# ouc-ocean-group/RRNet

Hardware: AMD Instinct MI355X
Metric: images/sec (train step) (higher is better)
Workload: dtype f32; 1 GPU; RRNet hourglass-104 (2 stacks) train step, 1024x1024 synthetic VisDrone frames, fp32; per_gpu_batch=8, global_batch=8, k=1500, parallelism=dp1

## Files before the change

include/rrnet_hip_wino.h:

```cpp
#ifndef RRNET_HIP_WINO_H
#define RRNET_HIP_WINO_H

#include <stddef.h>

#ifdef __cplusplus
extern "C" {
#endif

#ifndef __HIP_INCLUDE_HIP_HIP_RUNTIME_API_H__
#ifndef RRNET_HIP_H
typedef struct ihipStream_t *hipStream_t;
#endif
#endif

#define RR_WINO_PLAN_INTS 11
int rr_conv_wino_plan(int math, int n, int h, int wd, int c, int k, int r, int s, int stride, int pad_h, int pad_w, int out_h,
                      int out_w, int flags, int *plan);
size_t rr_conv_wino_ws_bytes(int n, int h, int wd, int c, int k);
int rr_wino_filter(const float *w, float *u, int k, int c, hipStream_t stream);
int rr_wino_filter_batch(const long long *table, int nfilters, hipStream_t stream);
int rr_conv_wino_fprop(const float *x, const float *u, const float *bias, float *y, double *stat_slab, float *ws, size_t ws_bytes,
                       int n, int h, int wd, int c, int k, int relu, int accumulate, hipStream_t stream);
int rr_conv_wino_dgrad_bnsum(const float *dy, const float *u, float *dx, float *ws, size_t ws_bytes, int n, int h, int wd, int c,
                             int k, int accumulate, const float *prod_y, const float *prod_z, const float *prod_mean,
                             const float *prod_invstd, const float *prod_mask_scale, const float *prod_mask_shift, double *slab,
                             double *sums, hipStream_t stream);
int rr_wino_input(const float *x, float *v, int n, int h, int wd, int c, hipStream_t stream);
int rr_wino_gemm(const float *v, const float *u, float *m, long tiles, int c, int k, hipStream_t stream);

#ifdef __cplusplus
}
#endif
#endif
```

rrnet_amd/csrc/conv.hip:

```cpp
#include "conv_launch.h"
#include <hip/amd_detail/amd_hip_unsafe_atomics.h>

namespace {

typedef float f32x4 __attribute__((ext_vector_type(4)));
typedef float f32x16 __attribute__((ext_vector_type(16)));

__device__ float rr_zero16[4] = {0.f, 0.f, 0.f, 0.f};

constexpr int BM = 128;
constexpr int BK = 32;

struct ConvArgs {
    const float *src;
    const float *w;
    float *dst;
    const float *bias;
    double *stat_slab;
    const float *bs_y, *bs_z, *bs_mean, *bs_invstd, *bs_msc, *bs_msh;
    int bs_relu_bias;
    int N;
    int SH, SW, SC;
    int DH, DW, DC;
    int R, S, stride, pad_h, pad_w;
// ... 673 lines not shown
#pragma unroll
            for (int w = 0; w < WM; ++w) {
                d1 += sred[(w * BN + t) * 2 + 0];
                d2 += sred[(w * BN + t) * 2 + 1];
            }
            double *slab = a.stat_slab + (long)m_tile * 2 * a.DC;
            slab[n0 + t] = d1;
            slab[a.DC + n0 + t] = d2;
        }
    }
}

struct WgradArgs {
    const float *x;
    const float *dy;
    float *dw;
    const float *zero;
    int N, H, W, C, K, R, S, P, Q, stride, pad_h, pad_w;
    int M;
    int chunks_per_split;
    int mt, nt;
    const int *gate;
    int gate_max;
};

template <int BMW, int BN, bool A_SCALAR, bool B_SCALAR, int PIPE>
__global__ __launch_bounds__(256, PIPE == 3 ? 3 : 1) void conv_wgrad_kernel(const WgradArgs a)
{
    static_assert(PIPE == 0 || PIPE == 1 || PIPE == 3, "conv_wgrad_kernel: PIPE 0, 1 or 3");
    if (a.gate != nullptr && *a.gate <= a.gate_max) return;
    constexpr int TILES = (BMW / 32) * (BN / 32);
    constexpr int KS = TILES == 1 ? 4 : 1;
    constexpr int WN = TILES == 16 ? 2 : (BN / 32 >= 4 ? 4 : 1);
    constexpr int WM = 4 / (WN * KS);
    constexpr int TM = BMW / (WM * 32);
    constexpr int TN = BN / (WN * 32);
    constexpr int A_ELEMS = BK * BMW, B_ELEMS = BK * BN;
    constexpr int TPR_A = BMW / 4, RPP_A = 256 / TPR_A, AJ = BMW / 32;
    constexpr int TPR_B = BN / 4, RPP_B = 256 / TPR_B, BJ = BN / 32;

    extern __shared__ __align__(16) float lds[];
    constexpr int NBUF = PIPE == 3 ? 1 : 2;
    float *As = lds, *Bs = lds + NBUF * A_ELEMS;

    const int t = threadIdx.x, lane = t & 63, wave = t >> 6;
    const int wk = KS > 1 ? wave : 0;
    const int wm = KS > 1 ? 0 : wave / WN, wn = KS > 1 ? 0 : wave % WN;
    const int RS = a.R * a.S;
    int logical = xcd_remap(blockIdx.x, gridDim.x);
    const int tap = logical % RS; logical /= RS;
    const int n_tile = logical % a.nt; logical /= a.nt;
    const int m_tile = logical % a.mt;
    const int split = logical / a.mt;
    const int r = tap / a.S, s = tap - r * a.S;
    const int ko0 = m_tile * BMW, c0 = n_tile * BN;
    const int total_chunks = (a.M + BK - 1) / BK;
    const int kc_begin = split * a.chunks_per_split;
    int kc_end = kc_begin + a.chunks_per_split;
    if (kc_end > total_chunks) kc_end = total_chunks;
    if (kc_begin >= kc_end) return;

    f32x4 ra[AJ], rb[BJ];
    const int a_row = t / TPR_A, a_col = (t % TPR_A) * 4;
    const int b_row = t / TPR_B, b_col = (t % TPR_B) * 4;

    int bn_[BJ], bp_[BJ], bq_[BJ];
#pragma unroll
    for (int j = 0; j < BJ; ++j) {
        const long m = (long)kc_begin * BK + b_row + RPP_B * j;
        const int pq = a.P * a.Q;
        bn_[j] = (int)(m / pq);
        const int rem = (int)(m - (long)bn_[j] * pq);
        bp_[j] = rem / a.Q;
        bq_[j] = rem - bp_[j] * a.Q;
    }
    const bool a_ko_ok = ko0 + a_col < a.K;
    const bool b_c_ok = c0 + b_col < a.C;
// ... 96 lines not shown
        for (int q = 0; q < 4; ++q) {
            const int kr = 2 * (4 * g + q) + lh;
#pragma unroll
            for (int i = 0; i < TM; ++i) fa[q][i] = A[kr * BMW + (wm * TM + i) * 32 + lr];
#pragma unroll
            for (int j = 0; j < TN; ++j) fb[q][j] = B[kr * BN + (wn * TN + j) * 32 + lr];
        }
    };
    auto sub = [&](const float (&fa)[4][TM], const float (&fb)[4][TN], int q) {
#pragma unroll
        for (int i = 0; i < TM; ++i)
#pragma unroll
            for (int j = 0; j < TN; ++j)
                acc[i][j] = __builtin_amdgcn_mfma_f32_32x32x2f32(fa[q][i], fb[q][j], acc[i][j], 0, 0, 0);
        __builtin_amdgcn_sched_barrier(0);
    };
    auto make_srd = [](const float *p, long bytes) {
        const unsigned long long u = reinterpret_cast<unsigned long long>(p);
        const unsigned lo = __builtin_amdgcn_readfirstlane((unsigned)u);
        const unsigned hi = __builtin_amdgcn_readfirstlane((unsigned)(u >> 32));
        void *q = reinterpret_cast<void *>(((unsigned long long)hi << 32) | lo);
        return __builtin_amdgcn_make_buffer_rsrc(q, 0, __builtin_amdgcn_readfirstlane((int)bytes), 0x00020000);
    };
    const __amdgpu_buffer_rsrc_t rs_dy = make_srd(a.dy, (long)a.M * a.K * 4);
    const long x_shift = ALIGNED ? (long)a.pad_w * a.C * 4 : 0;
    const __amdgpu_buffer_rsrc_t rs_x = make_srd(reinterpret_cast<const float *>(reinterpret_cast<const char *>(a.x) - x_shift),
                                                 (long)a.N * a.H * a.W * a.C * 4 + x_shift);
    constexpr unsigned OOB = 0xFFFFFFF0u;
    int a_off[AJ], a_m[AJ];
#pragma unroll
    for (int j = 0; j < AJ; ++j) {
        a_m[j] = a_row + RPP_A * j;
        a_off[j] = (a_m[j] * a.K + ko0 + a_col) * 4;
    }
    const int a_step = BK * a.K * 4;
    const int rr_off = r - a.pad_h, ss_off = s - a.pad_w;
    constexpr unsigned FAR = 0x80000000u;
    int s_n = 0, s_p = 0, s_q0 = 0;
    unsigned a_voff[AJ], b_voff[BJ];
    int b_iw0[BJ];
    if constexpr (ALIGNED) {
        const int m0 = kc_begin * BK, pq = a.P * a.Q;
        s_n = m0 / pq;
        const int rem = m0 - s_n * pq;
        s_p = rem / a.Q;
        s_q0 = rem - s_p * a.Q;
#pragma unroll
        for (int j = 0; j < AJ; ++j) a_voff[j] = a_ko_ok ? (unsigned)a_off[j] : FAR;
#pragma unroll
// ... 218 lines not shown
{
    const long M = (long)n * p * q;
    return (size_t)((M + BM - 1) / BM) * 2 * k * sizeof(double);
}

int rr_conv_wino_gemm(const float *v, const float *u, float *m, long tiles, int c, int k, hipStream_t stream, const char *name)
{
    RR_CHECK_ARG(tiles > 0 && c > 0 && k > 0 && c % 4 == 0 && k % 4 == 0 && tiles * c * 4 < (1l << 31) && tiles * k * 4 < (1l << 31)
                 && (long)k * c * 4 < (1l << 31), "%s: bad GEMM geometry", name);
    ConvArgs a{};
    a.src = v; a.w = u; a.dst = m; a.zero = zero_page();
    a.N = 1; a.SH = 1; a.SW = (int)tiles; a.SC = c;
    a.DH = 1; a.DW = (int)tiles; a.DC = k;
    a.R = 1; a.S = 1; a.stride = 1; a.ksplit = 1;
    a.M = (int)tiles; a.Kg = c; a.wK = k; a.wC = c; a.dst32 = 1;
    a.batch_src = tiles * c; a.batch_w = (long)k * c; a.batch_dst = tiles * k;
    const int bn = k > 64 ? 128 : 64;
    const dim3 grid(rr_cdiv(tiles, BM) * rr_cdiv(k, bn), 16, 1);
    if (bn == 128)
        return rr_launch(conv_igemm_kernel<128, 0, false, BK, 2, false, false, true>, grid, 256, igemm_lds(128, false, 1), stream, a, name);
    return rr_launch(conv_igemm_kernel<64, 0, false, BK, 2, false, false, true>, grid, 256, igemm_lds(64, false, 1), stream, a, name);
}

int rr_conv_colstats(const float *y, long M, int C, double *slab, hipStream_t stream, const char *name)
{
    const int lanes = 256 / (C / 4);
    int sblocks = rr_cdiv(M, (long)lanes * 8);
    if (sblocks > 256) sblocks = 256;
    hipLaunchKernelGGL(colstats_kernel, dim3(sblocks), dim3(256), 0, stream, y, M, C, slab);
    RR_CHECK_LAUNCH(name);
    return RR_OK;
}

static int fprop_impl(const char *name, const float *x, const float *w, const float *bias, float *y, double *stat_slab,
                      int n, int h, int wd, int c, int k, int r, int s, int stride, int pad_h,
                      int pad_w, int relu, int accumulate, hipStream_t stream, const BnSumArgs *bs = nullptr, const int *gate = nullptr,
                      int gate_max = 0)
{
    const rr_plan::FpropPlan pl = rr_plan::fprop_plan(rr_plan::MATH_F32, {n, h, wd, c, k, r, s, stride, pad_h, pad_w, 0, 0},
                                                      {bias != nullptr, relu != 0, stat_slab != nullptr, rr_conv_link(bs), accumulate != 0, false});
    RR_CHECK_ARG(pl.refuse == nullptr, "%s: %s", name, pl.refuse);
    RR_CHECK_ARG(gate == nullptr || (!pl.rows && !pl.pos_major && bs == nullptr && pl.after == rr_plan::AFTER_NONE && !pl.zero_slab),
                 "%s: this shape does not launch the plain forward kernel alone: no gate", name);
    if (pl.rows) return rr_conv1x1_rows(x, w, bias, y, pl.M, c, k, relu, stream);
    ConvArgs a{};
    a.gate = gate; a.gate_max = gate_max;
// ... 285 lines not shown
```

rrnet_amd/csrc/conv_launch.h:

```cpp
#pragma once
#include "common.h"
#include "conv_plan.h"
#include "rrnet_hip.h"
#include "rrnet_hip_rows.h"

struct BnSumArgs {
    const float *y, *z, *mean, *invstd, *msc, *msh;
    double *slab;
    double *sums;
    int relu_bias;
    bool bn_ok(int c) const { return y && mean && invstd && slab && sums && (!msc == !msh) && c % 4 == 0 && c <= 1024; }
    bool relu_bias_ok(int c, int k) const { return z && slab && sums && c % 4 == 0 && k % 4 == 0 && c <= 1024; }
    template <typename A> void into(A &a) const
    {
        a.stat_slab = slab; a.bs_y = y; a.bs_z = z; a.bs_mean = mean; a.bs_invstd = invstd; a.bs_msc = msc; a.bs_msh = msh; a.bs_relu_bias = relu_bias;
    }
};

template <typename K, typename A>
inline int rr_launch(K kern, dim3 grid, int threads, size_t lds, hipStream_t stream, const A &args, const char *name)
{
    if (lds > 48 * 1024)
        RR_CHECK_HIP(hipFuncSetAttribute(reinterpret_cast<const void *>(kern), hipFuncAttributeMaxDynamicSharedMemorySize, (int)lds), name);
    hipLaunchKernelGGL(kern, grid, dim3(threads), lds, stream, args);
    RR_CHECK_LAUNCH(name);
    return RR_OK;
}

inline int rr_refuse(const char *name, const rr_plan::Refusal &r)
{
    char why[256];
    snprintf(why, sizeof(why), r.why, r.a[0], r.a[1], r.a[2], r.a[3], r.a[4]);
    rr_set_error("%s: %s", name, why);
    return RR_ERR_ARG;
}

inline int rr_conv_link(const BnSumArgs *bs) { return bs == nullptr ? rr_plan::LINK_NONE : (bs->relu_bias ? rr_plan::LINK_RELU_BIAS : rr_plan::LINK_BN); }

int rr_conv_colstats(const float *y, long M, int C, double *slab, hipStream_t stream, const char *name);

int rr_conv_wino_gemm(const float *v, const float *u, float *m, long tiles, int c, int k, hipStream_t stream, const char *name);

int rr_gated_zero(float *p, size_t bytes, const int *count, int max_rows, int when_rows, hipStream_t stream, const char *name);

inline int rr_conv_before_launch(const rr_plan::FpropPlan &pl, int n, int k, float *y, double *stat_slab, hipStream_t stream, const char *name)
{
    RR_CHECK_HIP(rr_zero2(pl.zero_dst ? y : nullptr, pl.zero_dst ? sizeof(float) * (size_t)pl.M * k : 0, pl.zero_slab ? stat_slab : nullptr,
                          pl.zero_slab ? rr_conv_stat_slab_bytes(n, pl.dh, pl.dw, k) : 0, stream), name);
    return RR_OK;
}

inline int rr_conv_after_launch(const rr_plan::FpropPlan &pl, const BnSumArgs *bs, int k, const float *y, double *stat_slab, hipStream_t stream,
                                const char *name)
{
    switch (pl.after) {
    case rr_plan::AFTER_REDUCE_SLAB: return rr_bn_reduce_slab(bs->slab, rr_cdiv(pl.M, rr_plan::BM), k, bs->sums, stream);
    case rr_plan::AFTER_BWD_REDUCE: return rr_bn_bwd_reduce(y, bs->z, bs->y, bs->mean, bs->invstd, bs->msc, bs->msh, bs->sums, pl.M, k, 1, stream);
    case rr_plan::AFTER_COLSTATS: return rr_conv_colstats(y, pl.M, k, stat_slab, stream, name);
    default: return RR_OK;
    }
}

struct DgradS1Geom { int p, q, pad_h, pad_w; };
inline int rr_dgrad_s1_geom(const char *name, int h, int wd, int r, int s, int pad_h, int pad_w, bool producer_ok, DgradS1Geom *g)
// ... 56 lines not shown
```

rrnet_amd/csrc/conv_plan.h:

```cpp
#pragma once
#include <stdlib.h>

namespace rr_plan {

enum { MATH_F32 = 0, MATH_BF16 = 1, MATH_F16X3 = 2 };
enum { FAM_CONV16 = 3 };
enum { LINK_NONE = 0, LINK_BN = 1, LINK_RELU_BIAS = 2 };
enum { AFTER_NONE = 0, AFTER_REDUCE_SLAB = 1, AFTER_BWD_REDUCE = 2, AFTER_COLSTATS = 3 };

constexpr int BM = 128;
constexpr int BK = 32;

inline int cdiv(long a, long b) { return (int)((a + b - 1) / b); }

inline int mid_tiles() { return 48; }
inline int small_tiles() { return 16; }

inline int pick_ksplit(int blocks, int nk)
{
    static int enabled = -1;
    if (enabled < 0) {
        const char *e = getenv("RR_CONV_SPLITK");
        enabled = (e && atoi(e) == 0) ? 0 : 1;
    }
// ... 341 lines not shown
    RR_PLAN_REFUSE(math != MATH_F32, "fp32 arithmetic only");
    RR_PLAN_REFUSE(!(g.r == 3 && g.s == 3 && g.stride == 1 && g.pad_h == 1 && g.pad_w == 1), "3x3, stride 1, pad 1 only");
    RR_PLAN_REFUSE(g.out_h > 0 || g.out_w > 0, "no explicit output size");
    RR_PLAN_REFUSE(!(g.c % 4 == 0 && g.k % 4 == 0), "C and K must be multiples of 4");
    RR_PLAN_REFUSE(f.strided_dst, "no strided destination");
    RR_PLAN_REFUSE(f.link == LINK_RELU_BIAS, "the conv + bias + ReLU link is not built on this route");
    RR_PLAN_REFUSE(f.link == LINK_BN && (f.bias || f.relu || f.stats || g.k > 1024), "a BatchNorm link: plain data gradient, at most 1024 channels");
    const long M = (long)g.n * g.h * g.w;
    p.th = (g.h + 1) / 2; p.tw = (g.w + 1) / 2;
    p.tiles = (long)g.n * p.th * p.tw;
    RR_PLAN_REFUSE(!(M * g.c * 4 < G2 && M * g.k * 4 < G2 && 9l * g.c * g.k * 4 < G2 && p.tiles * g.c * 4 < G2 && p.tiles * g.k * 4 < G2),
                   "tensors must stay below 2 GiB");
    p.bn = g.k > 64 ? 128 : 64;
    p.gemm_blocks = cdiv(p.tiles, BM) * cdiv(g.k, p.bn);
    p.out_x = cdiv(M, BM);
    p.out_y = cdiv(g.k / 4, 64);
    p.tiles_per_wg = cdiv(p.tiles, p.out_x);
    p.ws_bytes = 16l * p.tiles * ((long)g.c + g.k) * 4;
    if (M < WINO_MIN_PIXELS) { p.refuse = "fewer output pixels than the route's floor"; p.floor_only = 1; }
#undef RR_PLAN_REFUSE
    return p;
}

}
```

rrnet_amd/csrc/conv_wino.hip:

```cpp
#include "conv_launch.h"
#include "rrnet_hip_wino.h"

namespace {

typedef float f32x4 __attribute__((ext_vector_type(4)));

__device__ __forceinline__ __amdgpu_buffer_rsrc_t wino_srd(const void *p, long bytes)
{
    const unsigned long long u = reinterpret_cast<unsigned long long>(p);
    const unsigned lo = __builtin_amdgcn_readfirstlane((unsigned)u);
    const unsigned hi = __builtin_amdgcn_readfirstlane((unsigned)(u >> 32));
    void *q = reinterpret_cast<void *>(((unsigned long long)hi << 32) | lo);
    return __builtin_amdgcn_make_buffer_rsrc(q, 0, __builtin_amdgcn_readfirstlane((int)bytes), 0x00020000);
}
constexpr unsigned OOB = 0xFFFFFFF0u;
__device__ __forceinline__ f32x4 wino_load(__amdgpu_buffer_rsrc_t rs, unsigned off)
{
    return __builtin_bit_cast(f32x4, __builtin_amdgcn_raw_buffer_load_b128(rs, off, 0, 0));
}

struct WinoFilterRow { const float *w; float *u; long K, C; };

__global__ __launch_bounds__(256) void wino_filter_kernel(const WinoFilterRow *table, const WinoFilterRow one)
{
// ... 46 lines not shown
#pragma unroll
            for (int j = 0; j < 4; ++j) {
                const int ih = h0 + i, iw = w0 + j;
                const bool in = (unsigned)ih < (unsigned)H && (unsigned)iw < (unsigned)W;
                const unsigned off = in ? (unsigned)((((n * H + ih) * W + iw) * C + c) * 4) : OOB;
                d[i][j] = wino_load(rs, off);
            }
        f32x4 m[4][4];
#pragma unroll
        for (int j = 0; j < 4; ++j) {
            m[0][j] = d[0][j] - d[2][j];
            m[1][j] = d[1][j] + d[2][j];
            m[2][j] = d[2][j] - d[1][j];
            m[3][j] = d[1][j] - d[3][j];
        }
        float *vp = v + t * C + c;
        const long bs = tiles * C;
#pragma unroll
        for (int a = 0; a < 4; ++a) {
            *reinterpret_cast<f32x4 *>(vp + (4 * a + 0) * bs) = m[a][0] - m[a][2];
            *reinterpret_cast<f32x4 *>(vp + (4 * a + 1) * bs) = m[a][1] + m[a][2];
            *reinterpret_cast<f32x4 *>(vp + (4 * a + 2) * bs) = m[a][2] - m[a][1];
            *reinterpret_cast<f32x4 *>(vp + (4 * a + 3) * bs) = m[a][1] - m[a][3];
        }
    }
}

struct WinoOutArgs {
    const float *m;
    float *y;
    const float *bias;
    double *slab;
    const float *bs_y, *bs_z, *bs_mean, *bs_invstd, *bs_msc, *bs_msh;
    int H, W, K, TH, TW;
    long tiles, y_bytes;
    int per_wg, relu, accumulate;
};

template <bool LINK>
__global__ __launch_bounds__(256) void wino_output_kernel(const WinoOutArgs a)
{
    __shared__ double sred[rr_plan::WINO_OUT_LANES][64][8];
    const int t = threadIdx.x, cl = t & 63, tl = t >> 6;
    const int c = (blockIdx.y * 64 + cl) * 4;
    const bool c_ok = c < a.K;
    const int cm = c_ok ? c : 0;
// ... 112 lines not shown
        for (int e = 0; e < 4; ++e) {
            double r1 = 0.0, r2 = 0.0;
#pragma unroll
            for (int l = 0; l < rr_plan::WINO_OUT_LANES; ++l) { r1 += sred[l][cl][e]; r2 += sred[l][cl][4 + e]; }
            row[c + e] = r1;
            row[a.K + c + e] = r2;
        }
    }
}

int grid_for(long threads)
{
    long blocks = (threads + 255) / 256;
    return (int)(blocks > 256 * 64 ? 256 * 64 : (blocks < 1 ? 1 : blocks));
}

int run_filter(const WinoFilterRow *table, const WinoFilterRow &one, int nfilters, int blocks_x, hipStream_t stream, const char *name)
{
    hipLaunchKernelGGL(wino_filter_kernel, dim3(blocks_x, nfilters), dim3(256), 0, stream, table, one);
    RR_CHECK_LAUNCH(name);
    return RR_OK;
}

int run_input(const float *x, float *v, int n, int h, int wd, int c, const rr_plan::WinoPlan &pl, hipStream_t stream, const char *name)
{
    hipLaunchKernelGGL(wino_input_kernel, dim3(grid_for(pl.tiles * (c / 4))), dim3(256), 0, stream, x, v, h, wd, c, pl.th, pl.tw, pl.tiles,
                       (long)n * h * wd * c * 4);
    RR_CHECK_LAUNCH(name);
    return RR_OK;
}

int checked_plan(const char *name, int n, int h, int wd, int c, int k, const rr_plan::ConvFlags &f, size_t ws_bytes, rr_plan::WinoPlan *pl)
{
    *pl = rr_plan::wino_plan(rr_plan::MATH_F32, {n, h, wd, c, k, 3, 3, 1, 1, 1, 0, 0}, f);
    RR_CHECK_ARG(pl->refuse == nullptr || pl->floor_only, "%s: %s", name, pl->refuse);
    RR_CHECK_ARG(ws_bytes >= (size_t)pl->ws_bytes, "%s: workspace of %ld bytes needed (rr_conv_wino_ws_bytes)", name, pl->ws_bytes);
    return RR_OK;
}

int run_route(const char *name, const float *x, const float *u, float *y, float *ws, int n, int h, int wd, int c, int k,
              const rr_plan::WinoPlan &pl, WinoOutArgs &o, bool link, hipStream_t stream)
{
    float *v = ws, *m = ws + 16 * pl.tiles * c;
    if (int rc = run_input(x, v, n, h, wd, c, pl, stream, name)) return rc;
    if (int rc = rr_conv_wino_gemm(v, u, m, pl.tiles, c, k, stream, name)) return rc;
    o.m = m; o.y = y; o.y_bytes = (long)n * h * wd * k * 4; o.H = h; o.W = wd; o.K = k; o.TH = pl.th; o.TW = pl.tw; o.tiles = pl.tiles; o.per_wg = pl.tiles_per_wg;
    if (link) hipLaunchKernelGGL(wino_output_kernel<true>, dim3(pl.out_x, pl.out_y), dim3(256), 0, stream, o);
    else hipLaunchKernelGGL(wino_output_kernel<false>, dim3(pl.out_x, pl.out_y), dim3(256), 0, stream, o);
    RR_CHECK_LAUNCH(name);
    return RR_OK;
}

}

extern "C" int rr_conv_wino_plan(int math, int n, int h, int wd, int c, int k, int r, int s, int stride, int pad_h, int pad_w, int out_h,
                                 int out_w, int flags, int *plan)
{
    RR_CHECK_ARG(plan != nullptr && ((flags >> 8) & 3) <= rr_plan::LINK_RELU_BIAS, "rr_conv_wino_plan: bad arguments");
    const rr_plan::WinoPlan pl = rr_plan::wino_plan(math, {n, h, wd, c, k, r, s, stride, pad_h, pad_w, out_h, out_w},
                                                    {(flags & 1) != 0, (flags & 2) != 0, (flags & 4) != 0, (flags >> 8) & 3, (flags & 8) != 0,
                                                     (flags & 16) != 0});
    const int out[RR_WINO_PLAN_INTS] = {pl.refuse == nullptr, pl.floor_only, (int)(pl.tiles & 0x7fffffff), (int)(pl.tiles >> 31), pl.bn, pl.gemm_blocks, pl.out_x,
                                        pl.out_y, pl.tiles_per_wg, (int)(pl.ws_bytes & 0x7fffffff), (int)(pl.ws_bytes >> 31)};
    for (int i = 0; i < RR_WINO_PLAN_INTS; ++i) plan[i] = out[i];
    return RR_OK;
}

// ... 2 lines not shown
    if (n <= 0 || h <= 0 || wd <= 0 || c <= 0 || k <= 0) return 0;
    return (size_t)16 * n * ((h + 1) / 2) * ((wd + 1) / 2) * ((size_t)c + k) * sizeof(float);
}

extern "C" int rr_wino_filter_batch(const long long *table, int nfilters, hipStream_t stream)
{
    static_assert(sizeof(WinoFilterRow) == 4 * sizeof(long long), "rr_wino_filter_batch: four 64-bit words per filter");
    RR_CHECK_ARG(table != nullptr && nfilters >= 0 && nfilters < 65536, "rr_wino_filter_batch: bad arguments");
    if (nfilters == 0) return RR_OK;
    return run_filter(reinterpret_cast<const WinoFilterRow *>(table), WinoFilterRow{}, nfilters, 64, stream, "rr_wino_filter_batch");
}

extern "C" int rr_wino_filter(const float *w, float *u, int k, int c, hipStream_t stream)
{
    RR_CHECK_ARG(w != nullptr && u != nullptr && k > 0 && c > 0, "rr_wino_filter: bad arguments");
    return run_filter(nullptr, WinoFilterRow{w, u, k, c}, 1, grid_for((long)k * c), stream, "rr_wino_filter");
}

extern "C" int rr_wino_input(const float *x, float *v, int n, int h, int wd, int c, hipStream_t stream)
{
    rr_plan::WinoPlan pl;
    if (int rc = checked_plan("rr_wino_input", n, h, wd, c, c, {}, (size_t)-1, &pl)) return rc;
    RR_CHECK_ARG(x != nullptr && v != nullptr, "rr_wino_input: null argument");
    return run_input(x, v, n, h, wd, c, pl, stream, "rr_wino_input");
}

extern "C" int rr_wino_gemm(const float *v, const float *u, float *m, long tiles, int c, int k, hipStream_t stream)
{
    RR_CHECK_ARG(v != nullptr && u != nullptr && m != nullptr, "rr_wino_gemm: null argument");
    return rr_conv_wino_gemm(v, u, m, tiles, c, k, stream, "rr_wino_gemm");
}

extern "C" int rr_conv_wino_fprop(const float *x, const float *u, const float *bias, float *y, double *stat_slab, float *ws, size_t ws_bytes,
                                  int n, int h, int wd, int c, int k, int relu, int accumulate, hipStream_t stream)
{
    rr_plan::WinoPlan pl;
    if (int rc = checked_plan("rr_conv_wino_fprop", n, h, wd, c, k,
                              {bias != nullptr, relu != 0, stat_slab != nullptr, rr_plan::LINK_NONE, accumulate != 0, false}, ws_bytes, &pl))
        return rc;
    RR_CHECK_ARG(x != nullptr && u != nullptr && y != nullptr && ws != nullptr, "rr_conv_wino_fprop: null argument");
    WinoOutArgs o{};
    o.bias = bias; o.slab = stat_slab; o.relu = relu != 0; o.accumulate = accumulate != 0;
    return run_route("rr_conv_wino_fprop", x, u, y, ws, n, h, wd, c, k, pl, o, false, stream);
}

extern "C" int rr_conv_wino_dgrad_bnsum(const float *dy, const float *u, float *dx, float *ws, size_t ws_bytes, int n, int h, int wd, int c,
                                        int k, int accumulate, const float *prod_y, const float *prod_z, const float *prod_mean,
                                        const float *prod_invstd, const float *prod_mask_scale, const float *prod_mask_shift, double *slab,
                                        double *sums, hipStream_t stream)
{
    const char *name = "rr_conv_wino_dgrad_bnsum";
    const BnSumArgs bs{prod_y, prod_z, prod_mean, prod_invstd, prod_mask_scale, prod_mask_shift, slab, sums, 0};
    RR_CHECK_ARG(bs.bn_ok(c) && dy != nullptr && u != nullptr && dx != nullptr && ws != nullptr,
                 "%s: bad arguments (every tensor, the producer's tensors and the two buffers; C %% 4 == 0, C <= 1024)", name);
    rr_plan::WinoPlan pl;
    if (int rc = checked_plan(name, n, h, wd, k, c, {false, false, false, rr_plan::LINK_BN, accumulate != 0, false}, ws_bytes, &pl)) return rc;
    WinoOutArgs o{};
    o.slab = slab; o.accumulate = accumulate != 0;
    o.bs_y = prod_y; o.bs_z = prod_z; o.bs_mean = prod_mean; o.bs_invstd = prod_invstd; o.bs_msc = prod_mask_scale; o.bs_msh = prod_mask_shift;
    if (int rc = run_route(name, dy, u, dx, ws, n, h, wd, k, c, pl, o, true, stream)) return rc;
    return rr_bn_reduce_slab(slab, pl.out_x, c, sums, stream);
}
```

rrnet_amd/ops.py:

```python
import os
import sys
import threading
import types
import weakref

import torch

from rrnet_amd import _C

CL = torch.channels_last


class KernelTimer:

    def __init__(self, only=None, every=1):
        self.records = []
        self.bytes = {}
        self.only = only
        self.every = max(int(every), 1)
        self.seen = {}

    def launch(self, name, flops, fn, detail=None, nbytes=0.0):
        if self.only is not None and name not in self.only:
            return fn()
# ... 628 lines not shown
        tail = (link.y, z if link.use_z else None, link.mean, link.invstd, link.msc, link.msh, slab, link.sums) + tail
    _launch(name, flops, "rr_conv_dgrad_s1" + sfx, (dy, wt, out) + geo + tail, geo[:7] + (1,),
            4.0 * (dy.numel() + out.numel() * ((2 if geo[9] else 1) + (link is not None)) + w.numel()))


def _dgrad_s2(dy, w, out, geo, flops, bf, conv16):
    src = bf16_of(dy) if conv16 else dy
    wsub = torch.empty(w.numel(), dtype=torch.bfloat16 if conv16 else torch.float32, device=dy.device)
    sfx, tag, tail = _math_call(bf, dy, w)
    _launch("conv16_dgrad_s2" if conv16 else "conv_dgrad_s2" + tag, flops, "rr_conv16_dgrad_s2" if conv16 else "rr_conv_dgrad_s2" + sfx,
            (src, w, out) + geo + (wsub,) + tail, geo[:7] + (2,))


def _dgrad_fp32(dy, w, out, geo, flops, stride):
    n, h, wd, c, k = geo[:5]
    _launch(_igemm_name("dgrad", c, (k % 4 != 0) or (c % 4 != 0), n * h * wd, stride), flops, "rr_conv_dgrad",
            (dy, w, out) + geo[:7] + (stride,) + geo[7:], geo[:7] + (stride,))


_WINO = _C.Family("rrnet_hip_wino.h")
_CONV_WINO = os.environ.get("RR_CONV_WINO", "1") != "0"
_WINO_BELOW_FLOOR = False
_WINO_TAKES = {}
_WINO_PLAN_FN = []
_WINO_WS = {}
FLAT_BUFFERS = weakref.WeakSet()


def wino_takes(n, h, wd, c, k, r, s, stride, pad, bias=False, relu=False, stats=False, accumulate=False, link=False):
    if not _CONV_WINO:
        return False
    key = (n, h, wd, c, k, r, s, stride, pad[0], pad[1], int(bias) | int(relu) << 1 | int(stats) << 2 | int(accumulate) << 3 | int(link) << 8)
    hit = _WINO_TAKES.get(key)
    if hit is None:
        if not _WINO_PLAN_FN:
            f, (sig, _) = getattr(_C.lib(), "rr_conv_wino_plan"), _C.declared("rr_conv_wino_plan")
            f.restype, f.argtypes = sig[0], sig[1]
            _WINO_PLAN_FN.append(f)
        plan = (_C.c_int * 11)()
        _C.check(_WINO_PLAN_FN[0](MATH_F32, *key[:10], 0, 0, key[10], plan), "rr_conv_wino_plan")
        hit = _WINO_TAKES[key] = (bool(plan[0]), bool(plan[1]))
    return hit[0] or (hit[1] and _WINO_BELOW_FLOOR)


def _wino_ws(device, n, h, wd, c, k):
    need = _WINO.call("rr_conv_wino_ws_bytes", n, h, wd, c, k) // 4
    key = (device, torch.cuda.current_stream(device).cuda_stream)
    ws = _WINO_WS.get(key)
    if ws is None or ws.numel() < need:
        _WINO_WS[key] = None
        ws = _WINO_WS[key] = torch.empty(need, dtype=torch.float32, device=device)
    return ws


def _wino_filter(w, flipped, wt=None):
    for flat in FLAT_BUFFERS:
        u = flat.wino_view(w, flipped)
        if u is not None:
            return u
    k, c = w.shape[0], w.shape[1]
    src = _flipped_filter(w, wt, None, False)[0] if flipped else w
    u = torch.empty(16 * k * c, dtype=torch.float32, device=w.device)
    _WINO.call("rr_wino_filter", src, u, *((c, k) if flipped else (k, c)))
    return u


def _dgrad_wino(dy, w, out, geo, flops, wt, link=None, z=None):
    n, h, wd, c, k = geo[:5]
    u, ws = _wino_filter(w, True, wt), _wino_ws(dy.device, n, h, wd, k, c)
    nbytes = 4.0 * (dy.numel() + out.numel() * ((2 if geo[9] else 1) + (link is not None)) + w.numel()) + 2.0 * ws.numel() * 4.0
    if link is None:
        _launch("conv_dgrad<wino>", flops * 16.0 / 36.0, "rr_conv_wino_fprop",
                (dy, u, None, out, None, ws, ws.numel() * 4, n, h, wd, k, c, 0, geo[9]), geo[:7] + (1,), nbytes, call=_WINO.call)
        return
    slab = torch.empty(_C.call("rr_conv_stat_slab_bytes", n, h, wd, c) // 8, dtype=torch.float64, device=dy.device)
    link.sums, link.dz = _ZEROS.take(2 * c, dy.device), out
    _launch("conv_dgrad<wino>+bnsum", flops * 16.0 / 36.0, "rr_conv_wino_dgrad_bnsum",
            (dy, u, out, ws, ws.numel() * 4, n, h, wd, c, k, geo[9], link.y, z if link.use_z else None, link.mean, link.invstd, link.msc,
             link.msh, slab, link.sums), geo[:7] + (1,), nbytes, call=_WINO.call)


_ROWS = _C.Family("rrnet_hip_rows.h")
_CONV_ROWS = os.environ.get("RR_CONV_ROWS", "1") != "0"
_ROWS_MAX_SHARE = 8
_TARGETS_MAX_SHARE = 4


# ... 73 lines not shown

def conv_wgrad(x, dy, dw, stride=1, pad=(0, 0), explicit_out=False, algo_c=None):
    _C.require_cuda(x, dy, dw)
    assert (is_nhwc(x) or is_phantom(x)) and (is_nhwc(dy) or is_phantom(dy)) and is_nhwc(dw)
    n, c, h, wd = x.shape
    k, c2, r, s = dw.shape
    assert c == c2 and dy.shape[1] == k
    flops = 2.0 * dy.shape[0] * dy.shape[2] * dy.shape[3] * k * (c * r * s if algo_c is None else algo_c)
    if wgrad16_takes(x.shape, dy.shape, dw.shape, stride) and not explicit_out:
        x16, dy16 = bf16_of(x), bf16_of(dy)
        _launch("conv16_wgrad", flops, "rr_conv16_wgrad", (x16, dy16, dw, n, h, wd, c, k, r, s, stride, pad[0], pad[1]),
                (n, h, wd, c, k, r, s, stride))
        return dw
    listed = rows_side.now(dy) if not explicit_out and not is_phantom(x) and not is_phantom(dy) else None
    if listed is not None and _rows_shape_ok(dy, tuple(x.shape), tuple(dw.shape), stride):
        rows, count = listed[:2]
        args = (x, dy, dw, n, h, wd, c, k, r, s, pad[0], pad[1])
        max_rows = n * h * wd // _ROWS_MAX_SHARE
        _launch("conv_wgrad<rows>", 0.0, "rr_conv_wgrad_rows", args + (rows, count, max_rows), (n, h, wd, c, k, r, s, 1), call=_ROWS.call)
        _launch("conv_wgrad<dense>", 0.0, "rr_conv_wgrad_unless", args + (count, max_rows), (n, h, wd, c, k, r, s, 1), call=_ROWS.call)
        return dw
    x, dy = f32_of(x), f32_of(dy)
    bf = _bf16_ok(c, k, r, s, x, dy, pixels=dy.shape[0] * dy.shape[2] * dy.shape[3]) if wgrad_16bit_shape(c, k, r, s) else 0
    sfx, tag, wtail = _math_call(bf, x, dy)
    _launch("conv_wgrad<BN=%d>%s" % (128 if c > 32 else 32, tag), flops, "rr_conv_wgrad" + sfx,
            (x, dy, dw, n, h, wd, c, k, r, s, stride, pad[0], pad[1]) + ((dy.shape[2], dy.shape[3]) if explicit_out else (0, 0)) + wtail,
            (n, h, wd, c, k, r, s, stride))
    return dw


def _f32(n, device):
    return torch.empty(n, dtype=torch.float32, device=device)


class _ZeroPool:

    CHUNK = 128 * 1024

    def __init__(self):
        self.buf = {}

    def take(self, n, device):
        n8 = (n + 1) // 2 * 2
        key = (device.type, device.index, torch.cuda.current_stream(device).cuda_stream if device.type == "cuda" else 0)
        cur = self.buf.get(key)
        if cur is None or cur[1] + n8 > cur[0].numel():
# ... 1577 lines not shown
```

Measured before the change: 21.48 images/sec.

## Add Winograd F(2x2,3x3) weight-gradient path for fp32 3x3 stride-1 convolutions

Adds a Winograd weight-gradient route for 3x3, stride-1, pad-1 fp32 convolutions. It transforms input tiles and output-gradient tiles into 16 transformed slices, runs a batched 16-slice GEMM through a BATCH variant of the existing wgrad kernel, then folds the 4x4 results back into 3x3 filter gradients with accumulation. The aim is to cut the multiply count of the dominant wgrad GEMMs, paid for with extra transform passes, a large workspace, a zero-fill, and possible fp32 rounding differences. It is on by default for layers with at least 64K pixels and C, K above 32.

```diff
diff --git a/include/rrnet_hip_wino.h b/include/rrnet_hip_wino.h
--- a/include/rrnet_hip_wino.h
+++ b/include/rrnet_hip_wino.h
@@ -27,6 +27,15 @@
                              double *sums, hipStream_t stream);
 int rr_wino_input(const float *x, float *v, int n, int h, int wd, int c, hipStream_t stream);
 int rr_wino_gemm(const float *v, const float *u, float *m, long tiles, int c, int k, hipStream_t stream);
+#define RR_WINO_WGRAD_PLAN_INTS 10
+int rr_conv_wino_wgrad_plan(int math, int n, int h, int wd, int c, int k, int r, int s, int stride, int pad_h, int pad_w, int out_h,
+                            int out_w, int flags, int *plan);
+size_t rr_conv_wino_wgrad_ws_bytes(int n, int h, int wd, int c, int k);
+int rr_conv_wino_wgrad(const float *x, const float *dy, float *dw, float *ws, size_t ws_bytes, int n, int h, int wd, int c, int k,
+                       hipStream_t stream);
+int rr_wino_dy(const float *dy, float *w, int n, int h, int wd, int k, hipStream_t stream);
+int rr_wino_wgrad_gemm(const float *v, const float *w, float *s, long tiles, int c, int k, hipStream_t stream);
+int rr_wino_dw(const float *s, float *dw, int k, int c, hipStream_t stream);
 
 #ifdef __cplusplus
 }
diff --git a/rrnet_amd/csrc/conv.hip b/rrnet_amd/csrc/conv.hip
--- a/rrnet_amd/csrc/conv.hip
+++ b/rrnet_amd/csrc/conv.hip
@@ -719,12 +719,14 @@
     int mt, nt;
     const int *gate;
     int gate_max;
+    long slice_x, slice_dy;
 };
 
-template <int BMW, int BN, bool A_SCALAR, bool B_SCALAR, int PIPE>
+template <int BMW, int BN, bool A_SCALAR, bool B_SCALAR, int PIPE, bool BATCH = false>
 __global__ __launch_bounds__(256, PIPE == 3 ? 3 : 1) void conv_wgrad_kernel(const WgradArgs a)
 {
     static_assert(PIPE == 0 || PIPE == 1 || PIPE == 3, "conv_wgrad_kernel: PIPE 0, 1 or 3");
+    static_assert(!BATCH || (PIPE != 0 && BMW == 128 && BN == 128 && !A_SCALAR && !B_SCALAR), "conv_wgrad_kernel: BATCH on the pipelined 128x128 kernels");
     if (a.gate != nullptr && *a.gate <= a.gate_max) return;
     constexpr int TILES = (BMW / 32) * (BN / 32);
     constexpr int KS = TILES == 1 ? 4 : 1;
@@ -743,13 +745,21 @@
     const int t = threadIdx.x, lane = t & 63, wave = t >> 6;
     const int wk = KS > 1 ? wave : 0;
     const int wm = KS > 1 ? 0 : wave / WN, wn = KS > 1 ? 0 : wave % WN;
-    const int RS = a.R * a.S;
+    const int RS = BATCH ? 16 : a.R * a.S;
     int logical = xcd_remap(blockIdx.x, gridDim.x);
-    const int tap = logical % RS; logical /= RS;
-    const int n_tile = logical % a.nt; logical /= a.nt;
-    const int m_tile = logical % a.mt;
-    const int split = logical / a.mt;
-    const int r = tap / a.S, s = tap - r * a.S;
+    int tap, n_tile, m_tile, split;
+    if constexpr (BATCH) {
+        n_tile = logical % a.nt; logical /= a.nt;
+        m_tile = logical % a.mt; logical /= a.mt;
+        tap = logical % RS;
+        split = logical / RS;
+    } else {
+        tap = logical % RS; logical /= RS;
+        n_tile = logical % a.nt; logical /= a.nt;
+        m_tile = logical % a.mt;
+        split = logical / a.mt;
+    }
+    const int r = BATCH ? 0 : tap / a.S, s = BATCH ? 0 : tap - r * a.S;
     const int ko0 = m_tile * BMW, c0 = n_tile * BN;
     const int total_chunks = (a.M + BK - 1) / BK;
     const int kc_begin = split * a.chunks_per_split;
@@ -892,9 +902,9 @@
         void *q = reinterpret_cast<void *>(((unsigned long long)hi << 32) | lo);
         return __builtin_amdgcn_make_buffer_rsrc(q, 0, __builtin_amdgcn_readfirstlane((int)bytes), 0x00020000);
     };
-    const __amdgpu_buffer_rsrc_t rs_dy = make_srd(a.dy, (long)a.M * a.K * 4);
+    const __amdgpu_buffer_rsrc_t rs_dy = make_srd(BATCH ? a.dy + (long)tap * a.slice_dy : a.dy, (long)a.M * a.K * 4);
     const long x_shift = ALIGNED ? (long)a.pad_w * a.C * 4 : 0;
-    const __amdgpu_buffer_rsrc_t rs_x = make_srd(reinterpret_cast<const float *>(reinterpret_cast<const char *>(a.x) - x_shift),
+    const __amdgpu_buffer_rsrc_t rs_x = make_srd(reinterpret_cast<const float *>(reinterpret_cast<const char *>(BATCH ? a.x + (long)tap * a.slice_x : a.x) - x_shift),
                                                  (long)a.N * a.H * a.W * a.C * 4 + x_shift);
     constexpr unsigned OOB = 0xFFFFFFF0u;
     int a_off[AJ], a_m[AJ];
@@ -1159,6 +1169,21 @@
     return rr_launch(conv_igemm_kernel<64, 0, false, BK, 2, false, false, true>, grid, 256, igemm_lds(64, false, 1), stream, a, name);
 }
 
+int rr_conv_wino_wgrad_gemm(const float *v, const float *w, float *s, long tiles, int c, int k, hipStream_t stream, const char *name)
+{
+    RR_CHECK_ARG(tiles > 0 && c > 32 && k > 32 && c % 4 == 0 && k % 4 == 0 && tiles * c * 4 < (1l << 31) && tiles * k * 4 < (1l << 31)
+                 && 16l * k * c * 4 < (1l << 31), "%s: bad GEMM geometry", name);
+    const rr_plan::WinoWgradGemm pl = rr_plan::wino_wgrad_gemm_plan(tiles, c, k);
+    WgradArgs a{};
+    a.x = v; a.dy = w; a.dw = s; a.zero = zero_page();
+    a.N = 1; a.H = 1; a.W = (int)tiles; a.C = c; a.K = k; a.R = 1; a.S = 1;
+    a.P = 1; a.Q = (int)tiles; a.stride = 1;
+    a.M = (int)tiles; a.mt = pl.mt; a.nt = pl.nt; a.chunks_per_split = pl.per_split;
+    a.slice_x = tiles * c; a.slice_dy = tiles * k;
+    if (pl.pipe == 3) return rr_launch(conv_wgrad_kernel<128, 128, false, false, 3, true>, dim3(pl.grid), 256, pl.lds, stream, a, name);
+    return rr_launch(conv_wgrad_kernel<128, 128, false, false, 1, true>, dim3(pl.grid), 256, pl.lds, stream, a, name);
+}
+
 int rr_conv_colstats(const float *y, long M, int C, double *slab, hipStream_t stream, const char *name)
 {
     const int lanes = 256 / (C / 4);
diff --git a/rrnet_amd/csrc/conv_launch.h b/rrnet_amd/csrc/conv_launch.h
--- a/rrnet_amd/csrc/conv_launch.h
+++ b/rrnet_amd/csrc/conv_launch.h
@@ -40,6 +40,8 @@
 int rr_conv_colstats(const float *y, long M, int C, double *slab, hipStream_t stream, const char *name);
 
 int rr_conv_wino_gemm(const float *v, const float *u, float *m, long tiles, int c, int k, hipStream_t stream, const char *name);
+
+int rr_conv_wino_wgrad_gemm(const float *v, const float *w, float *s, long tiles, int c, int k, hipStream_t stream, const char *name);
 
 int rr_gated_zero(float *p, size_t bytes, const int *count, int max_rows, int when_rows, hipStream_t stream, const char *name);
 
diff --git a/rrnet_amd/csrc/conv_plan.h b/rrnet_amd/csrc/conv_plan.h
--- a/rrnet_amd/csrc/conv_plan.h
+++ b/rrnet_amd/csrc/conv_plan.h
@@ -387,4 +387,51 @@
     return p;
 }
 
-}
+constexpr long WINO_WGRAD_MIN_PIXELS = 65536;
+
+struct WinoWgradGemm { int mt, nt, pipe, splits, per_split, grid, lds; };
+inline WinoWgradGemm wino_wgrad_gemm_plan(long tiles, int c, int k)
+{
+    WinoWgradGemm p{};
+    p.mt = cdiv(k, 128); p.nt = cdiv(c, 128);
+    p.pipe = tiles % BK == 0 ? 3 : 1;
+    const WgradFill fill = p.pipe == 3 ? WGRAD_F32_PIPE3 : WGRAD_F32;
+    p.splits = pixel_splits(p.mt * p.nt * 16, cdiv(tiles, BK), fill.slots, fill.min_chunks, &p.per_split);
+    p.grid = p.mt * p.nt * 16 * p.splits;
+    p.lds = 4 * (p.pipe == 3 ? 1 : 2) * (BK * 128 + BK * 128);
+    return p;
+}
+
+struct WinoWgradPlan {
+    const char *refuse;
+    int floor_only;
+    int th, tw;
+    long tiles;
+    WinoWgradGemm gemm;
+    long ws_bytes;
+};
+
+inline WinoWgradPlan wino_wgrad_plan(int math, const ConvGeom &g, bool gated)
+{
+    WinoWgradPlan p{};
+    const long G2 = 1l << 31;
+#define RR_PLAN_REFUSE(cond, why) do { if (cond) { p.refuse = why; return p; } } while (0)
+    RR_PLAN_REFUSE(!(g.n > 0 && g.h > 0 && g.w > 0 && g.c > 0 && g.k > 0), "bad dims");
+    RR_PLAN_REFUSE(math != MATH_F32, "fp32 arithmetic only");
+    RR_PLAN_REFUSE(!(g.r == 3 && g.s == 3 && g.stride == 1 && g.pad_h == 1 && g.pad_w == 1), "3x3, stride 1, pad 1 only");
+    RR_PLAN_REFUSE(g.out_h > 0 || g.out_w > 0, "no explicit output size");
+    RR_PLAN_REFUSE(!(g.c % 4 == 0 && g.k % 4 == 0 && g.c > 32 && g.k > 32), "C and K must be multiples of 4 above 32");
+    RR_PLAN_REFUSE(gated, "no gated launch");
+    const long M = (long)g.n * g.h * g.w;
+    p.th = (g.h + 1) / 2; p.tw = (g.w + 1) / 2;
+    p.tiles = (long)g.n * p.th * p.tw;
+    RR_PLAN_REFUSE(!(M * g.c * 4 < G2 && M * g.k * 4 < G2 && 16l * g.c * g.k * 4 < G2 && p.tiles * g.c * 4 < G2 && p.tiles * g.k * 4 < G2),
+                   "tensors must stay below 2 GiB");
+    p.gemm = wino_wgrad_gemm_plan(p.tiles, g.c, g.k);
+    p.ws_bytes = (16l * p.tiles * ((long)g.c + g.k) + 16l * g.k * g.c) * 4;
+    if (M < WINO_WGRAD_MIN_PIXELS) { p.refuse = "fewer pixels than the route's floor"; p.floor_only = 1; }
+#undef RR_PLAN_REFUSE
+    return p;
+}
+
+}
diff --git a/rrnet_amd/csrc/conv_wino.hip b/rrnet_amd/csrc/conv_wino.hip
--- a/rrnet_amd/csrc/conv_wino.hip
+++ b/rrnet_amd/csrc/conv_wino.hip
@@ -92,6 +92,78 @@
             *reinterpret_cast<f32x4 *>(vp + (4 * a + 1) * bs) = m[a][1] + m[a][2];
             *reinterpret_cast<f32x4 *>(vp + (4 * a + 2) * bs) = m[a][2] - m[a][1];
             *reinterpret_cast<f32x4 *>(vp + (4 * a + 3) * bs) = m[a][1] - m[a][3];
+        }
+    }
+}
+
+__global__ __launch_bounds__(256) void wino_dy_kernel(const float *dy, float *w, int H, int W, int K, int TH, int TW, long tiles, long dy_bytes)
+{
+    const __amdgpu_buffer_rsrc_t rs = wino_srd(dy, dy_bytes);
+    const int K4 = K / 4;
+    const long total = tiles * K4;
+    for (long idx = (long)blockIdx.x * 256 + threadIdx.x; idx < total; idx += (long)gridDim.x * 256) {
+        const long t = idx / K4;
+        const int k = (int)(idx - t * K4) * 4;
+        const int tw = (int)(t % TW);
+        const long rest = t / TW;
+        const int th = (int)(rest % TH);
+        const int n = (int)(rest / TH);
+        f32x4 d[2][2];
+#pragma unroll
+        for (int i = 0; i < 2; ++i)
+#pragma unroll
+            for (int j = 0; j < 2; ++j) {
+                const int oh = 2 * th + i, ow = 2 * tw + j;
+                const bool in = oh < H && ow < W;
+                const unsigned off = in ? (unsigned)((((n * H + oh) * W + ow) * K + k) * 4) : OOB;
+                d[i][j] = wino_load(rs, off);
+            }
+        f32x4 m[4][2];
+#pragma unroll
+        for (int j = 0; j < 2; ++j) {
+            m[0][j] = d[0][j];
+            m[1][j] = d[0][j] + d[1][j];
+            m[2][j] = d[0][j] - d[1][j];
+            m[3][j] = -d[1][j];
+        }
+        float *wp = w + t * K + k;
+        const long bs = tiles * K;
+#pragma unroll
+        for (int a = 0; a < 4; ++a) {
+            *reinterpret_cast<f32x4 *>(wp + (4 * a + 0) * bs) = m[a][0];
+            *reinterpret_cast<f32x4 *>(wp + (4 * a + 1) * bs) = m[a][0] + m[a][1];
+            *reinterpret_cast<f32x4 *>(wp + (4 * a + 2) * bs) = m[a][0] - m[a][1];
+            *reinterpret_cast<f32x4 *>(wp + (4 * a + 3) * bs) = -m[a][1];
+        }
+    }
+}
+
+__global__ __launch_bounds__(256) void wino_dw_kernel(const float *s, float *dw, int K, int C)
+{
+    const int C4 = C / 4;
+    const long total = (long)K * C4;
+    for (long idx = (long)blockIdx.x * 256 + threadIdx.x; idx < total; idx += (long)gridDim.x * 256) {
+        const long ko = idx / C4;
+        const int c = (int)(idx - ko * C4) * 4;
+        const float *sp = s + ko * 16 * C + c;
+        f32x4 S[4][4], t[3][4];
+#pragma unroll
+        for (int i = 0; i < 16; ++i) S[i >> 2][i & 3] = *reinterpret_cast<const f32x4 *>(sp + (long)i * C);
+#pragma unroll
+        for (int b = 0; b < 4; ++b) {
+            t[0][b] = S[0][b] + 0.5f * (S[1][b] + S[2][b]);
+            t[1][b] = 0.5f * (S[1][b] - S[2][b]);
+            t[2][b] = 0.5f * (S[1][b] + S[2][b]) + S[3][b];
+        }
+        float *dp = dw + ko * 9 * C + c;
+#pragma unroll
+        for (int r = 0; r < 3; ++r) {
+            f32x4 *d0 = reinterpret_cast<f32x4 *>(dp + (long)(3 * r + 0) * C);
+            f32x4 *d1 = reinterpret_cast<f32x4 *>(dp + (long)(3 * r + 1) * C);
+            f32x4 *d2 = reinterpret_cast<f32x4 *>(dp + (long)(3 * r + 2) * C);
+            *d0 += t[r][0] + 0.5f * (t[r][1] + t[r][2]);
+            *d1 += 0.5f * (t[r][1] - t[r][2]);
+            *d2 += 0.5f * (t[r][1] + t[r][2]) + t[r][3];
         }
     }
 }
@@ -250,11 +322,34 @@
     return RR_OK;
 }
 
-int run_input(const float *x, float *v, int n, int h, int wd, int c, const rr_plan::WinoPlan &pl, hipStream_t stream, const char *name)
-{
-    hipLaunchKernelGGL(wino_input_kernel, dim3(grid_for(pl.tiles * (c / 4))), dim3(256), 0, stream, x, v, h, wd, c, pl.th, pl.tw, pl.tiles,
+int run_input(const float *x, float *v, int n, int h, int wd, int c, int th, int tw, long tiles, hipStream_t stream, const char *name)
+{
+    hipLaunchKernelGGL(wino_input_kernel, dim3(grid_for(tiles * (c / 4))), dim3(256), 0, stream, x, v, h, wd, c, th, tw, tiles,
                        (long)n * h * wd * c * 4);
     RR_CHECK_LAUNCH(name);
+    return RR_OK;
+}
+
+int run_dy(const float *dy, float *w, int n, int h, int wd, int k, int th, int tw, long tiles, hipStream_t stream, const char *name)
+{
+    hipLaunchKernelGGL(wino_dy_kernel, dim3(grid_for(tiles * (k / 4))), dim3(256), 0, stream, dy, w, h, wd, k, th, tw, tiles,
+                       (long)n * h * wd * k * 4);
+    RR_CHECK_LAUNCH(name);
+    return RR_OK;
+}
+
+int run_dw(const float *s, float *dw, int k, int c, hipStream_t stream, const char *name)
+{
+    hipLaunchKernelGGL(wino_dw_kernel, dim3(grid_for((long)k * (c / 4))), dim3(256), 0, stream, s, dw, k, c);
+    RR_CHECK_LAUNCH(name);
+    return RR_OK;
+}
+
+int checked_wgrad_plan(const char *name, int n, int h, int wd, int c, int k, size_t ws_bytes, rr_plan::WinoWgradPlan *pl)
+{
+    *pl = rr_plan::wino_wgrad_plan(rr_plan::MATH_F32, {n, h, wd, c, k, 3, 3, 1, 1, 1, 0, 0}, false);
+    RR_CHECK_ARG(pl->refuse == nullptr || pl->floor_only, "%s: %s", name, pl->refuse);
+    RR_CHECK_ARG(ws_bytes >= (size_t)pl->ws_bytes, "%s: workspace of %ld bytes needed (rr_conv_wino_wgrad_ws_bytes)", name, pl->ws_bytes);
     return RR_OK;
 }
 
@@ -270,7 +365,7 @@
               const rr_plan::WinoPlan &pl, WinoOutArgs &o, bool link, hipStream_t stream)
 {
     float *v = ws, *m = ws + 16 * pl.tiles * c;
-    if (int rc = run_input(x, v, n, h, wd, c, pl, stream, name)) return rc;
+    if (int rc = run_input(x, v, n, h, wd, c, pl.th, pl.tw, pl.tiles, stream, name)) return rc;
     if (int rc = rr_conv_wino_gemm(v, u, m, pl.tiles, c, k, stream, name)) return rc;
     o.m = m; o.y = y; o.y_bytes = (long)n * h * wd * k * 4; o.H = h; o.W = wd; o.K = k; o.TH = pl.th; o.TW = pl.tw; o.tiles = pl.tiles; o.per_wg = pl.tiles_per_wg;
     if (link) hipLaunchKernelGGL(wino_output_kernel<true>, dim3(pl.out_x, pl.out_y), dim3(256), 0, stream, o);
@@ -319,7 +414,7 @@
     rr_plan::WinoPlan pl;
     if (int rc = checked_plan("rr_wino_input", n, h, wd, c, c, {}, (size_t)-1, &pl)) return rc;
     RR_CHECK_ARG(x != nullptr && v != nullptr, "rr_wino_input: null argument");
-    return run_input(x, v, n, h, wd, c, pl, stream, "rr_wino_input");
+    return run_input(x, v, n, h, wd, c, pl.th, pl.tw, pl.tiles, stream, "rr_wino_input");
 }
 
 extern "C" int rr_wino_gemm(const float *v, const float *u, float *m, long tiles, int c, int k, hipStream_t stream)
@@ -358,3 +453,55 @@
     if (int rc = run_route(name, dy, u, dx, ws, n, h, wd, k, c, pl, o, true, stream)) return rc;
     return rr_bn_reduce_slab(slab, pl.out_x, c, sums, stream);
 }
+
+extern "C" int rr_conv_wino_wgrad_plan(int math, int n, int h, int wd, int c, int k, int r, int s, int stride, int pad_h, int pad_w, int out_h,
+                                       int out_w, int flags, int *plan)
+{
+    RR_CHECK_ARG(plan != nullptr, "rr_conv_wino_wgrad_plan: bad arguments");
+    const rr_plan::WinoWgradPlan pl = rr_plan::wino_wgrad_plan(math, {n, h, wd, c, k, r, s, stride, pad_h, pad_w, out_h, out_w}, (flags & 1) != 0);
+    const int out[RR_WINO_WGRAD_PLAN_INTS] = {pl.refuse == nullptr, pl.floor_only, (int)(pl.tiles & 0x7fffffff), (int)(pl.tiles >> 31), pl.gemm.pipe,
+                                              pl.gemm.splits, pl.gemm.per_split, pl.gemm.grid, (int)(pl.ws_bytes & 0x7fffffff), (int)(pl.ws_bytes >> 31)};
+    for (int i = 0; i < RR_WINO_WGRAD_PLAN_INTS; ++i) plan[i] = out[i];
+    return RR_OK;
+}
+
+extern "C" size_t rr_conv_wino_wgrad_ws_bytes(int n, int h, int wd, int c, int k)
+{
+    if (n <= 0 || h <= 0 || wd <= 0 || c <= 0 || k <= 0) return 0;
+    return ((size_t)16 * n * ((h + 1) / 2) * ((wd + 1) / 2) * ((size_t)c + k) + (size_t)16 * k * c) * sizeof(float);
+}
+
+extern "C" int rr_wino_dy(const float *dy, float *w, int n, int h, int wd, int k, hipStream_t stream)
+{
+    rr_plan::WinoWgradPlan pl;
+    if (int rc = checked_wgrad_plan("rr_wino_dy", n, h, wd, k, k, (size_t)-1, &pl)) return rc;
+    RR_CHECK_ARG(dy != nullptr && w != nullptr, "rr_wino_dy: null argument");
+    return run_dy(dy, w, n, h, wd, k, pl.th, pl.tw, pl.tiles, stream, "rr_wino_dy");
+}
+
+extern "C" int rr_wino_wgrad_gemm(const float *v, const float *w, float *s, long tiles, int c, int k, hipStream_t stream)
+{
+    RR_CHECK_ARG(v != nullptr && w != nullptr && s != nullptr, "rr_wino_wgrad_gemm: null argument");
+    return rr_conv_wino_wgrad_gemm(v, w, s, tiles, c, k, stream, "rr_wino_wgrad_gemm");
+}
+
+extern "C" int rr_wino_dw(const float *s, float *dw, int k, int c, hipStream_t stream)
+{
+    RR_CHECK_ARG(s != nullptr && dw != nullptr && k > 0 && c > 0 && c % 4 == 0, "rr_wino_dw: bad arguments");
+    return run_dw(s, dw, k, c, stream, "rr_wino_dw");
+}
+
+extern "C" int rr_conv_wino_wgrad(const float *x, const float *dy, float *dw, float *ws, size_t ws_bytes, int n, int h, int wd, int c, int k,
+                                  hipStream_t stream)
+{
+    const char *name = "rr_conv_wino_wgrad";
+    rr_plan::WinoWgradPlan pl;
+    if (int rc = checked_wgrad_plan(name, n, h, wd, c, k, ws_bytes, &pl)) return rc;
+    RR_CHECK_ARG(x != nullptr && dy != nullptr && dw != nullptr && ws != nullptr, "%s: null argument", name);
+    float *v = ws, *w = v + 16 * pl.tiles * c, *s = w + 16 * pl.tiles * k;
+    if (int rc = run_input(x, v, n, h, wd, c, pl.th, pl.tw, pl.tiles, stream, name)) return rc;
+    if (int rc = run_dy(dy, w, n, h, wd, k, pl.th, pl.tw, pl.tiles, stream, name)) return rc;
+    RR_CHECK_HIP(rr_zero2(s, sizeof(float) * 16 * (size_t)k * c, nullptr, 0, stream), name);
+    if (int rc = rr_conv_wino_wgrad_gemm(v, w, s, pl.tiles, c, k, stream, name)) return rc;
+    return run_dw(s, dw, k, c, stream, name);
+}
diff --git a/rrnet_amd/ops.py b/rrnet_amd/ops.py
--- a/rrnet_amd/ops.py
+++ b/rrnet_amd/ops.py
@@ -674,7 +674,7 @@
 _CONV_WINO = os.environ.get("RR_CONV_WINO", "1") != "0"
 _WINO_BELOW_FLOOR = False
 _WINO_TAKES = {}
-_WINO_PLAN_FN = []
+_WINO_PLAN_FN = {}
 _WINO_WS = {}
 FLAT_BUFFERS = weakref.WeakSet()
 
@@ -685,18 +685,23 @@
     key = (n, h, wd, c, k, r, s, stride, pad[0], pad[1], int(bias) | int(relu) << 1 | int(stats) << 2 | int(accumulate) << 3 | int(link) << 8)
     hit = _WINO_TAKES.get(key)
     if hit is None:
-        if not _WINO_PLAN_FN:
-            f, (sig, _) = getattr(_C.lib(), "rr_conv_wino_plan"), _C.declared("rr_conv_wino_plan")
-            f.restype, f.argtypes = sig[0], sig[1]
-            _WINO_PLAN_FN.append(f)
         plan = (_C.c_int * 11)()
-        _C.check(_WINO_PLAN_FN[0](MATH_F32, *key[:10], 0, 0, key[10], plan), "rr_conv_wino_plan")
+        _C.check(_wino_plan_fn("rr_conv_wino_plan")(MATH_F32, *key[:10], 0, 0, key[10], plan), "rr_conv_wino_plan")
         hit = _WINO_TAKES[key] = (bool(plan[0]), bool(plan[1]))
     return hit[0] or (hit[1] and _WINO_BELOW_FLOOR)
 
 
-def _wino_ws(device, n, h, wd, c, k):
-    need = _WINO.call("rr_conv_wino_ws_bytes", n, h, wd, c, k) // 4
+def _wino_plan_fn(entry):
+    f = _WINO_PLAN_FN.get(entry)
+    if f is None:
+        f, (sig, _) = getattr(_C.lib(), entry), _C.declared(entry)
+        f.restype, f.argtypes = sig[0], sig[1]
+        _WINO_PLAN_FN[entry] = f
+    return f
+
+
+def _wino_ws(device, n, h, wd, c, k, entry="rr_conv_wino_ws_bytes"):
+    need = _WINO.call(entry, n, h, wd, c, k) // 4
     key = (device, torch.cuda.current_stream(device).cuda_stream)
     ws = _WINO_WS.get(key)
     if ws is None or ws.numel() < need:
@@ -715,6 +720,23 @@
     u = torch.empty(16 * k * c, dtype=torch.float32, device=w.device)
     _WINO.call("rr_wino_filter", src, u, *((c, k) if flipped else (k, c)))
     return u
+
+
+_CONV_WINO_WGRAD = os.environ.get("RR_CONV_WINO_WGRAD", "1") != "0"
+_WINO_WGRAD_BELOW_FLOOR = False
+_WINO_WGRAD_TAKES = {}
+
+
+def wino_wgrad_takes(n, h, wd, c, k, r, s, stride, pad, explicit_out=False, gated=False):
+    if not _CONV_WINO_WGRAD or explicit_out:
+        return False
+    key = (n, h, wd, c, k, r, s, stride, pad[0], pad[1], 0, 0, int(gated))
+    hit = _WINO_WGRAD_TAKES.get(key)
+    if hit is None:
+        plan = (_C.c_int * 10)()
+        _C.check(_wino_plan_fn("rr_conv_wino_wgrad_plan")(MATH_F32, *key, plan), "rr_conv_wino_wgrad_plan")
+        hit = _WINO_WGRAD_TAKES[key] = (bool(plan[0]), bool(plan[1]))
+    return hit[0] or (hit[1] and _WINO_WGRAD_BELOW_FLOOR)
 
 
 def _dgrad_wino(dy, w, out, geo, flops, wt, link=None, z=None):
@@ -834,6 +856,13 @@
         return dw
     x, dy = f32_of(x), f32_of(dy)
     bf = _bf16_ok(c, k, r, s, x, dy, pixels=dy.shape[0] * dy.shape[2] * dy.shape[3]) if wgrad_16bit_shape(c, k, r, s) else 0
+    if bf == MATH_F32 and wino_wgrad_takes(n, h, wd, c, k, r, s, stride, pad, explicit_out):
+        ws = _wino_ws(x.device, n, h, wd, c, k, "rr_conv_wino_wgrad_ws_bytes")
+        tiles = n * ((h + 1) // 2) * ((wd + 1) // 2)
+        used = 4.0 * (16 * tiles * (c + k) + 16 * k * c)
+        _launch("conv_wgrad<wino>", flops * 16.0 / 36.0, "rr_conv_wino_wgrad", (x, dy, dw, ws, ws.numel() * 4, n, h, wd, c, k),
+                (n, h, wd, c, k, r, s, stride), 4.0 * (x.numel() + dy.numel() + 2 * dw.numel()) + 2.0 * used, call=_WINO.call)
+        return dw
     sfx, tag, wtail = _math_call(bf, x, dy)
     _launch("conv_wgrad<BN=%d>%s" % (128 if c > 32 else 32, tag), flops, "rr_conv_wgrad" + sfx,
             (x, dy, dw, n, h, wd, c, k, r, s, stride, pad[0], pad[1]) + ((dy.shape[2], dy.shape[3]) if explicit_out else (0, 0)) + wtail,
```

Result: faster. 22.52 images/sec, median of 6 (+4.9%).
